# mvenouziou/Boosted_DETR

Measured on AMD Instinct MI355X. Metric: images/sec training step (fwd+matcher+loss+bwd), 640x640 N=100, higher is better.
Workload: dtype f32 (conv/GEMM products as 3 split-f16 [fwd] / split-bf16 [grad] MFMA products, f32 accumulate)

## Files before the change

boosted_detr_amd/_lib.py:

```python
from __future__ import annotations

import ctypes as C
import os
from pathlib import Path

_LIB_PATH = Path(os.environ.get("BDETR_LIB") or Path(__file__).resolve().parent / "csrc" / "libbdetr.so")
_lib = None

c_f32p = C.c_void_p
c_i32p = C.c_void_p
c_i64p = C.c_void_p
c_stream = C.c_void_p


class ConvDesc(C.Structure):
    _fields_ = [(n, C.c_int) for n in ("N", "H", "W", "C", "K", "R", "S", "stride", "pad", "OH", "OW")]


class GemmDesc(C.Structure):
    _fields_ = [
        ("I", C.c_int), ("J", C.c_int), ("R", C.c_int), ("nb0", C.c_int), ("nb1", C.c_int),
        ("a", C.c_void_p), ("lda", C.c_int64), ("sa0", C.c_int64), ("sa1", C.c_int64), ("a_rcontig", C.c_int),
        ("b", C.c_void_p), ("ldb", C.c_int64), ("sb0", C.c_int64), ("sb1", C.c_int64), ("b_rcontig", C.c_int),
        ("c", C.c_void_p), ("ldc", C.c_int64), ("sc0", C.c_int64), ("sc1", C.c_int64),
# ... 101 lines not shown
    "bdetr_debug_checksum": (I, [P, L, P, P, P, I, U64, P]),
    "bdetr_graph_node_census": (I, [P, P, I]),
    "bdetr_bn_stats_fold_rows": (I, []),
    "bdetr_bn_stats_frozen": (I, [P, P, I, F, P, P, P]),
    "bdetr_bn_apply": (I, [P, P, P, P, P, P, I, P, L, I, P]),
    "bdetr_bn_bwd_chunks": (I, [L]),
    "bdetr_bn_bwd": (I, [P, P, P, P, P, P, P, I, I, P, P, P, P, P, L, I, P]),
    "bdetr_bn_rows_stats": (I, [P, I, L, I, F, P, P, P, P, P]),
    "bdetr_bn_rows_apply": (I, [P, P, P, P, P, P, I, L, I, I, P, F, P, P, P, P]),
    "bdetr_bn_rows_bwd": (I, [P, P, P, P, P, I, I, P, P, P, P, I, L, I, P]),
    "bdetr_maxpool3x3s2_fwd": (I, [P, P, I, I, I, I, I, I, P]),
    "bdetr_maxpool3x3s2_bwd": (I, [P, P, P, P, I, I, I, I, I, I, P]),
    "bdetr_stem_pool_bwd_chunks": (I, [L]),
    "bdetr_stem_pool_fwd": (I, [P, P, P, P, P, I, I, I, I, P, P, P, P, P]),
    "bdetr_stem_pool_bwd": (I, [P, P, P, P, P, P, P, I, I, I, I, P, I, P, P, P, P]),
    "bdetr_p16_s2d_pack_bf16": (I, [P, I, I, I, P, P]),
    "bdetr_p16_stem_bwd_weight": (I, [P, P, P, I, I, I, I, P]),
    "bdetr_p16_s2d_unpack_dw": (I, [P, P, I, P]),
    "bdetr_attention_head_dim": (I, []),
    "bdetr_attention_fwd": (I, [P, P, P, P, P, I, I, I, I, F, P]),
    "bdetr_attention_bwd": (I, [P, P, P, P, P, P, P, P, P, P, I, I, I, I, F, P]),
    "bdetr_softmax_rows_fwd": (I, [P, P, L, I, F, P]),
    "bdetr_softmax_rows_bwd": (I, [P, P, P, L, I, F, P]),
    "bdetr_add_dropout_layernorm_fwd": (I, [P, P, P, P, P, P, P, L, I, F, F, U64, P, P]),
    "bdetr_ln_bwd_chunks": (I, [L]),
    "bdetr_add_dropout_layernorm_bwd": (I, [P, P, P, P, P, P, P, P, P, P, P, L, I, F, U64, P, I, P]),
    "bdetr_rowchain_fwd": (I, [C.POINTER(RowchainFwdDesc), P]),
    "bdetr_rowchain_bwd": (I, [C.POINTER(RowchainBwdDesc), P]),
    "bdetr_rowchain_reduce": (I, [P, I, C.POINTER(C.c_void_p * 7), C.POINTER(C.c_int * 7), P]),
    "bdetr_rowchain_width": (I, []),
# ... 88 lines not shown
```

boosted_detr_amd/build.py:

```python
from __future__ import annotations

import hashlib
import os
import subprocess
import sys
from concurrent.futures import ThreadPoolExecutor
from pathlib import Path

CSRC = Path(__file__).resolve().parent / "csrc"
LIB = CSRC / "libbdetr.so"
OBJ_DIR = CSRC / "_obj"
SOURCES = ["common.cpp", "igemm.hip", "sgemm.hip", "hconv.hip", "hwgrad.hip", "p16.hip", "attention.hip", "rowchain.hip", "augment.hip", "norm.hip", "groupnorm_rows.hip", "elementwise.hip", "panoptic.hip", "matcher.hip", "optim.hip", "detmetric.hip", "maskmetric.hip", "maskraster.hip", "maskimage.hip", "panopticmerge.hip"]
ARCH = "gfx950"
COMMON_FLAGS = ["-O3", "-fPIC", f"--offload-arch={ARCH}", "-std=c++20", "-Wall", "-Wno-unused-function"] + os.environ.get("BDETR_CXXFLAGS", "").split()
PER_FILE_FLAGS = {"matcher.hip": ["-ffp-contract=off"], "detmetric.hip": ["-ffp-contract=off"], "maskmetric.hip": ["-ffp-contract=off"],
                  "maskraster.hip": ["-ffp-contract=off"], "maskimage.hip": ["-ffp-contract=off"], "panopticmerge.hip": ["-ffp-contract=off"]}


def _hipcc() -> str:
    for cand in (os.environ.get("HIPCC"), "/opt/rocm/bin/hipcc", "hipcc"):
        if cand and (os.path.isabs(cand) and os.path.exists(cand) or not os.path.isabs(cand)):
            return cand
    raise RuntimeError("hipcc not found")


def _digest(paths) -> str:
    h = hashlib.sha256()
    for p in sorted(paths):
        h.update(p.name.encode())
        h.update(p.read_bytes())
    return h.hexdigest()


def build(force: bool = False, verbose: bool = True) -> Path:
    deps = [CSRC / s for s in SOURCES] + [CSRC / "common.h", CSRC / "gemm_common.h", CSRC / "p16.h", CSRC.parent.parent / "include" / "bdetr.h"]
    stamp = CSRC / "_obj" / "stamp"
    dig = _digest(deps) + "|" + " ".join(COMMON_FLAGS)
    if not force and LIB.exists() and stamp.exists() and stamp.read_text() == dig:
        return LIB
    OBJ_DIR.mkdir(exist_ok=True)
    hipcc = _hipcc()

    headers = [d for d in deps if d.suffix == ".h"]

    def compile_one(src: str) -> Path:
        obj = OBJ_DIR / (src.rsplit(".", 1)[0] + ".o")
        flags = COMMON_FLAGS + PER_FILE_FLAGS.get(src, [])
        ostamp = OBJ_DIR / (src + ".stamp")
        odig = _digest([CSRC / src] + headers) + "|" + " ".join(flags)
        if not force and obj.exists() and ostamp.exists() and ostamp.read_text() == odig:
# ... 22 lines not shown
```

boosted_detr_amd/csrc/norm.hip:

```cpp
#include "common.h"
#include "p16.h"

namespace {

struct ColGeom { int tx, ty, gx; };
inline ColGeom col_geom(int C) {
    int c4 = C / 4;
    int tx = 1; while (tx < c4 && tx < 64) tx <<= 1;
    ColGeom g; g.tx = tx; g.ty = 256 / tx; g.gx = (c4 + tx - 1) / tx; return g;
}

template <class F>
__global__ __launch_bounds__(256) void colreduce2_kernel(F f, int64_t rows, int C, int tx, int64_t rows_per_chunk,
                                                         float* __restrict__ pa, float* __restrict__ pb) {
    __shared__ f32x4 sa[256], sb[256];
    const int tid = threadIdx.x;
    const int cx = tid % tx, ry = tid / tx, ty = 256 / tx;
    const int c = (blockIdx.x * tx + cx) * 4;
    const int64_t r0 = (int64_t)blockIdx.y * rows_per_chunk;
    const int64_t r1 = min(rows, r0 + rows_per_chunk);
    f32x4 a = {0, 0, 0, 0}, b = {0, 0, 0, 0};
    if (c < C) {
        int64_t r = r0 + ry;
        for (; r + ty < r1; r += 2 * ty) {
// ... 176 lines not shown
void sum_partials2(const float* pa, const float* pb, int nparts, int C, float* oa, float* ob, hipStream_t st) {
    if (nparts >= wide_reduce_min() && C % 4 == 0 && (reinterpret_cast<uintptr_t>(pa) | reinterpret_cast<uintptr_t>(pb)) % 16 == 0)
        hipLaunchKernelGGL(reduce_partials2_kernel<false>, dim3(C / 4), dim3(256), 0, st, pa, pb, nparts, C, oa, ob, BnFinalizeArgs{});
    else
        hipLaunchKernelGGL(sum_partials2_kernel, dim3((C + 7) / 8), dim3(256), 0, st, pa, pb, nparts, C, oa, ob);
}

struct StatFn {
    const float* x; int C;
    __device__ __forceinline__ void operator()(int64_t r, int c, f32x4& a, f32x4& b) const {
        f32x4 v = *reinterpret_cast<const f32x4*>(x + r * C + c);
        a = v; b = v * v;
    }
};

__device__ __forceinline__ float bn_affine(float v, float m, float rs, float g, float b) { return __builtin_fmaf(v - m, rs * g, b); }
__device__ __forceinline__ float bn_bwd_dx(float g, float xv, float m, float rs, float gm, float dg, float db, float inv_rows) {
    const float xh = (xv - m) * rs;
    const float t = __builtin_fmaf(-db, inv_rows, g);
    return __builtin_fmaf(-xh, dg * inv_rows, t) * (rs * gm);
}

__device__ __forceinline__ unsigned relu_mask_bits4(const void* mask, int64_t i) {
    const unsigned long long* w = reinterpret_cast<const unsigned long long*>(mask) + (i >> 6) * 4;
    const int b = (int)(i & 63);
    return (unsigned)((w[0] >> b) & 1ull) | ((unsigned)((w[1] >> b) & 1ull) << 1) | ((unsigned)((w[2] >> b) & 1ull) << 2) | ((unsigned)((w[3] >> b) & 1ull) << 3);
}

struct BnBwdFn {
    const float* dout; const float* out; const float* x; const float* mean; const float* rstd; const float* gamma; const float* beta;
    int C; int relu;
    int out_p16 = 0;
    int even_h = 0, even_w = 0;
    int dout_compact = 0;
    __device__ __forceinline__ void operator()(int64_t r, int c, f32x4& a, f32x4& b) const {
        const int64_t rg = r;
// ... 71 lines not shown
            }
        }
        if (dres != nullptr) reinterpret_cast<f32x4*>(dres)[i] = g;
        f32x4 r;
        if (frozen) {
            r = g * (rs * gm);
        } else {
            f32x4 dg = *reinterpret_cast<const f32x4*>(dgamma + c), db = *reinterpret_cast<const f32x4*>(dbeta + c);
#pragma unroll
            for (int e = 0; e < 4; ++e) r[e] = bn_bwd_dx(g[e], xv[e], m[e], rs[e], gm[e], dg[e], db[e], inv_rows);
        }
        reinterpret_cast<f32x4*>(dx)[i] = r;
    }
}

struct StemGeom { int N, H, W, C, PH, PW; };

__global__ __launch_bounds__(256) void stem_pool_fwd_kernel(const float* __restrict__ y, const float* __restrict__ mean, const float* __restrict__ rstd,
                                                            const float* __restrict__ gamma, const float* __restrict__ beta, StemGeom s,
                                                            float* __restrict__ out32, void* __restrict__ out_f16, unsigned* __restrict__ tap,
                                                            int* __restrict__ overflow_flag) {
    const int c4n = s.C / 4;
    const int64_t n4 = (int64_t)s.N * s.PH * s.PW * c4n;
    for (int64_t i = (int64_t)blockIdx.x * blockDim.x + threadIdx.x; i < n4; i += (int64_t)gridDim.x * blockDim.x) {
        const int c4 = (int)(i % c4n); unsigned t = (unsigned)(i / c4n);
        const int pw = (int)(t % (unsigned)s.PW); t /= (unsigned)s.PW; const int ph = (int)(t % (unsigned)s.PH); const int n = (int)(t / (unsigned)s.PH);
        const int c = c4 * 4;
        const f32x4 m = *reinterpret_cast<const f32x4*>(mean + c), rs = *reinterpret_cast<const f32x4*>(rstd + c);
        const f32x4 g = *reinterpret_cast<const f32x4*>(gamma + c), b = *reinterpret_cast<const f32x4*>(beta + c);
        f32x4 v[9];
        bool in[9];
// ... 13 lines not shown
            for (int e = 0; e < 4; ++e) {
                const float a = fmaxf(bn_affine(v[k][e], m[e], rs[e], g[e], b[e]), 0.f);
                if (a > mx[e]) { mx[e] = a; arg = (arg & ~(0xFFu << (8 * e))) | ((unsigned)k << (8 * e)); }
            }
        }
        tap[i] = arg;
        if (out32 != nullptr) reinterpret_cast<f32x4*>(out32)[i] = mx;
        if (out_f16 != nullptr) {
            p16_store4<true>(out_f16, i, mx[0], mx[1], mx[2], mx[3]);
            if (overflow_flag != nullptr) {
                const float top = fmaxf(fmaxf(mx[0], mx[1]), fmaxf(mx[2], mx[3]));
                if (!(top < P16_F16_LIMIT)) *overflow_flag = 1;
            }
        }
    }
}

__device__ __forceinline__ f32x4 stem_pixel_grad(const float* __restrict__ dpool, const unsigned* __restrict__ tap, const StemGeom& s, unsigned px, int c,
                                                 const f32x4 yv, const f32x4 m, const f32x4 rs, const f32x4 gm, const f32x4 bt, f32x4& xhat) {
    const int c4n = s.C / 4, c4 = c / 4;
    const int iw = (int)(px % (unsigned)s.W); const unsigned t = px / (unsigned)s.W;
    const int ih = (int)(t % (unsigned)s.H), n = (int)(t / (unsigned)s.H);
    const int ph0 = ih >> 1, pw0 = iw >> 1;
    const bool two_h = (ih & 1) & (int)(ph0 + 1 < s.PH), two_w = (iw & 1) & (int)(pw0 + 1 < s.PW);
    unsigned word[4];
    f32x4 dv[4];
    unsigned mine[4];
#pragma unroll
    for (int k = 0; k < 4; ++k) {
        const int a = k >> 1, b = k & 1;
        const bool real = (a == 0 || two_h) && (b == 0 || two_w);
        const int ph = ph0 + (a & (int)two_h), pw = pw0 + (b & (int)two_w);
        const int64_t o = (((int64_t)n * s.PH + ph) * s.PW + pw) * c4n + c4;
        mine[k] = real ? (unsigned)((ih - (ph * 2 - 1)) * 3 + (iw - (pw * 2 - 1))) : 0xFFu;
        word[k] = tap[o];
        dv[k] = reinterpret_cast<const f32x4*>(dpool)[o];
    }
    f32x4 g = {0.f, 0.f, 0.f, 0.f};
#pragma unroll
    for (int k = 0; k < 4; ++k)
#pragma unroll
        for (int e = 0; e < 4; ++e) if (((word[k] >> (8 * e)) & 0xFFu) == mine[k]) g[e] += dv[k][e];
    xhat = (yv - m) * rs;
#pragma unroll
    for (int e = 0; e < 4; ++e) if (!(bn_affine(yv[e], m[e], rs[e], gm[e], bt[e]) > 0.f)) g[e] = 0.f;
    return g;
}

struct StemBwdFn {
    const float* dpool; const unsigned* tap; const float* y; const float* mean; const float* rstd; const float* gamma; const float* beta; StemGeom s;
    __device__ __forceinline__ void operator()(int64_t r, int c, f32x4& a, f32x4& b) const {
        const f32x4 yv = *reinterpret_cast<const f32x4*>(y + r * s.C + c);
        const f32x4 m = *reinterpret_cast<const f32x4*>(mean + c), rs = *reinterpret_cast<const f32x4*>(rstd + c);
        const f32x4 gm = *reinterpret_cast<const f32x4*>(gamma + c), bt = *reinterpret_cast<const f32x4*>(beta + c);
        f32x4 xh;
        a = stem_pixel_grad(dpool, tap, s, (unsigned)r, c, yv, m, rs, gm, bt, xh);
        b = a * xh;
    }
};

__global__ __launch_bounds__(256) void stem_bwd_apply_kernel(const float* __restrict__ dpool, const unsigned* __restrict__ tap, const float* __restrict__ y,
// ... 463 lines not shown
    const StemGeom s{N, H, W, C, (H + 2 - 3) / 2 + 1, (W + 2 - 3) / 2 + 1};
    const int64_t rows = (int64_t)N * H * W;
    ColGeom g = col_geom(C);
    int64_t rpc = chunk_rows_for(rows, STEM_BWD_CHUNKS, 64);
    int nch = (int)cdiv64(rows, rpc);
    float* pa = ws; float* pb = ws + (int64_t)nch * C;
    StemBwdFn f{dpool, reinterpret_cast<const unsigned*>(tap), y, mean, rstd, gamma, beta, s};
    hipLaunchKernelGGL((colreduce2_kernel<StemBwdFn>), dim3(g.gx, nch), dim3(256), 0, st, f, rows, C, g.tx, rpc, pa, pb);
    sum_partials2(pa, pb, nch, C, dbeta, dgamma, st);
    const int64_t n4 = rows * C / 4;
    hipLaunchKernelGGL(stem_bwd_apply_kernel, dim3(ew_grid(n4, 256, 2)), dim3(256), 0, st, dpool, reinterpret_cast<const unsigned*>(tap), y, mean, rstd, gamma, beta,
                       dgamma, dbeta, s, dy, dy_p16, n4, 1.0f / (float)rows);
    return bdetr_launch_status("stem_pool_bwd");
}

static int channel_aligned_grid(int64_t n4, int C) {
    int grid = ew_grid(n4, 256, 2);
    int a = C / 4, b = 256;
    while (b) { const int t = a % b; a = b; b = t; }
    const int mult = (C / 4) / a;
    if (mult > 1 && mult <= 8) grid = (grid + mult - 1) / mult * mult;
    return grid;
}

extern "C" int bdetr_bn_apply_p16(const float* x, const float* mean, const float* rstd, const float* gamma,
                                  const float* beta, const void* residual, int residual_p16, const bdetr_bn_affine* residual_bn, int relu,
                                  float* out32, void* out_f16, void* out_bf16,
                                  uint64_t* relu_mask, int* overflow_flag, int64_t rows, int C, void* stream) {
    BDETR_CHECK_ARG(x && mean && rstd && gamma && beta && (out32 || out_f16 || out_bf16) && rows > 0 && C > 0 && C % 8 == 0,
                    "bdetr_bn_apply_p16: bad arguments (C %% 8 == 0 required)");
// ... 142 lines not shown
```

boosted_detr_amd/kernels.py:

```python
from __future__ import annotations

import ctypes as C
from dataclasses import dataclass
from typing import Optional, Tuple

import numpy as np
import torch

from . import _lib
from ._lib import BnAffine, BnBwdFuse, ConvDesc, GemmDesc, LossDesc, RowchainBwdDesc, RowchainFwdDesc, check

ACT_NONE, ACT_RELU, ACT_TANH = 0, 1, 2


_LAUNCH_STREAM = [None]


def set_launch_stream(handle: Optional[int]) -> Optional[int]:
    prev = _LAUNCH_STREAM[0]
    _LAUNCH_STREAM[0] = handle
    return prev


GEMM_FP32, GEMM_BF16X3, GEMM_MIXED, GEMM_SPLIT, GEMM_BF16X6 = 0, 1, 2, 3, 4
# ... 663 lines not shown
                                _p(ws), _stream()), "stem_pool_bwd")
    return dy, dgamma, dbeta


def stem_bwd_weight_s2d(x4, dy_bf16, dw):
    _chk(x4, dy_bf16, dw)
    L = _lib.lib()
    N, H, W, Cc = x4.shape
    Kout = dw.shape[0]
    assert Cc == 4 and H % 2 == 0 and W % 2 == 0 and tuple(dw.shape) == (Kout, 7, 7, 4) and tuple(dy_bf16.shape) == (N, H // 2, W // 2, Kout)
    x2 = empty(N, H // 2, W // 2, 16, like=x4)
    check(L.bdetr_p16_s2d_pack_bf16(_p(x4), N, H, W, _p(x2), _stream()), "p16_s2d_pack_bf16")
    dw2 = empty(Kout, 4, 4, 16, like=x4)
    check(L.bdetr_zero(_p(dw2), dw2.numel(), _stream()), "zero")
    check(L.bdetr_p16_stem_bwd_weight(_p(x2), _p(dy_bf16), _p(dw2), N, H // 2, W // 2, Kout, _stream()), "p16_stem_bwd_weight")
    check(L.bdetr_p16_s2d_unpack_dw(_p(dw2), _p(dw), Kout, _stream()), "p16_s2d_unpack_dw")
    return dw


def attention_fwd(q, k, v, heads, scale):
    _chk(q, k, v)
    B, nq, D = q.shape
    nk = k.shape[1]
    o = empty(B, heads, nq, D // heads, like=q)
    lse = empty(B, heads, nq, like=q)
    check(_lib.lib().bdetr_attention_fwd(_p(q), _p(k), _p(v), _p(o), _p(lse), B, heads, nq, nk, scale, _stream()), "attention_fwd")
    return o, lse


def attention_bwd(q, k, v, o, d_o, lse, heads, scale):
# ... 779 lines not shown
```

boosted_detr_amd/ops.py:

```python
from __future__ import annotations

import math
import os
import weakref
from typing import Optional

import numpy as np
import torch

from . import kernels as K
from . import _lib
from .engine import WEIGHTS_VERSION, Variable, capture, current_tape, dense_contribution, info, materialise, own, side_task, tag

_dropout_site = [0]
_dropout_seed_dev = [None]


def dropout_seed_tensor() -> torch.Tensor:
    if _dropout_seed_dev[0] is None:
        _dropout_seed_dev[0] = torch.full((1,), 0x5EED, dtype=torch.int64, device="cuda")
    return _dropout_seed_dev[0]


def set_dropout_seed(seed: int, write: bool = True) -> None:
# ... 471 lines not shown
        g, mine = g.contiguous(), info(g).owned
        return tuple(own(g[l * B:(l + 1) * B]) if mine else g[l * B:(l + 1) * B] for l in range(L))

    _rec([out], list(xs), backward)
    return out


def maxpool(x: torch.Tensor) -> torch.Tensor:
    y = K.maxpool_fwd(x)
    _rec([y], [x], lambda g: (own(K.maxpool_bwd(x, y, g.contiguous())),))
    return y


STEM_FUSE = os.environ.get("BDETR_STEM_FUSE", "1") != "0"
STEM_S2D = os.environ.get("BDETR_STEM_S2D", "1") != "0"


def conv_bn_relu_maxpool(x: torch.Tensor, w: Variable, b: Variable, bn: BNState, stride: int, pad: int, training: bool,
                         bn_batch_stats: bool) -> torch.Tensor:
    N, H, W, Cin = x.shape
    Kout, R, S, _ = w.value.shape
    if not (STEM_FUSE and training and bn_batch_stats and _p16_active() and Kout % 8 == 0):
        return maxpool(conv_bn(x, w, b, bn, stride, pad, True, training=training, bn_batch_stats=bn_batch_stats, x_needs_grad=False))
    g = K.ConvGeom(N, H, W, Cin, Kout, R, S, stride, pad)
    x32 = as_fp32(x)
    y, parts = K.conv2d_fwd(x32, w.value, b.value, g, K.ACT_NONE, want_stats=True)
    if parts is None or parts[0] is None:
        parts = K.colstats(_2d(y))
    mean, rstd = K.bn_stats(g.M, Kout, parts, bn.eps, bn.momentum, True, bn.moving_mean.value, bn.moving_var.value, like=y)
    _, out, tap = K.stem_pool_fwd(y, mean, rstd, bn.gamma.value, bn.beta.value)
    attach_packed(out, out.detach(), p16_only=True)

    def backward(g_out):
        sg, sb = GradSink(bn.gamma), GradSink(bn.beta)
        s2d = (STEM_S2D and w.needs_grad and (R, S, stride, pad, Cin) == (7, 7, 2, 3, 4) and H % 2 == 0 and W % 2 == 0 and Kout % 64 == 0
               and K.get_gemm_precision() in ("split", "mixed") and not K.deterministic())
        dy, _, _ = K.stem_pool_bwd(materialise(g_out).contiguous(), tap, y, mean, rstd, bn.gamma.value, bn.beta.value, dgamma=sg.buf, dbeta=sb.buf,
                                   dy_p16=s2d)
        sg.commit()
        sb.commit()
        if s2d:
            _param_grads_task(w, b, lambda dw, pz: K.stem_bwd_weight_s2d(x32, dy, dw), None, x32, dy)
        else:
            _param_grads_task(w, b, lambda dw, pz: K.conv2d_bwd_weight(x32, dy, g, dw=dw, prezeroed=pz), None, x32, dy)
        return (None,)

    _rec([out], [x], backward)
    return out


def dense(x: torch.Tensor, w: Variable, b: Variable, act: int = K.ACT_NONE) -> torch.Tensor:
# ... 285 lines not shown
```

include/bdetr.h:

```cpp
#ifndef BDETR_H
#define BDETR_H
#include <stdint.h>
#ifdef __cplusplus
extern "C" {
#endif

#define BDETR_ABI_VERSION 8

int         bdetr_abi_version(void);
const char* bdetr_last_error(void);
int         bdetr_device_cus(void);

int         bdetr_low_priority_stream_create(void** stream_out);
int         bdetr_stream_priority_range(int* least, int* greatest);
int         bdetr_side_stream_candidates(void* main_stream, int ncand, int loads, int ticks, void** streams_out, float* scores_ms, float* unloaded_ms);
int         bdetr_stream_destroy(void* stream);

enum { BDETR_GEMM_FP32 = 0, BDETR_GEMM_BF16X3 = 1, BDETR_GEMM_MIXED = 2, BDETR_GEMM_SPLIT = 3, BDETR_GEMM_BF16X6 = 4 };
int         bdetr_set_gemm_precision(int mode);
int         bdetr_get_gemm_precision(void);

int bdetr_prof_enable(int on);
int bdetr_prof_read(double* total_ms, int64_t* launches, double* flops);
int bdetr_prof_read_arith(int arith, double* total_ms, int64_t* launches, double* flops);
// ... 128 lines not shown
                      int grouped_stats, int frozen, float* dx, float* dgamma, float* dbeta, float* ws, int G, int64_t R, int C,
                      void* stream);

int bdetr_maxpool3x3s2_fwd(const float* x, float* y, int N, int H, int W, int C, int OH, int OW, void* stream);
int bdetr_maxpool3x3s2_bwd(const float* x, const float* y, const float* dy, float* dx,
                           int N, int H, int W, int C, int OH, int OW, void* stream);

int bdetr_stem_pool_bwd_chunks(int64_t rows);
int bdetr_stem_pool_fwd(const float* y, const float* mean, const float* rstd, const float* gamma, const float* beta,
                        int N, int H, int W, int C, float* out32, void* out_f16, uint8_t* tap, int* overflow_flag, void* stream);
int bdetr_stem_pool_bwd(const float* dpool, const uint8_t* tap, const float* y, const float* mean, const float* rstd, const float* gamma,
                        const float* beta, int N, int H, int W, int C, float* dy, int dy_p16 , float* dgamma, float* dbeta, float* ws, void* stream);
int bdetr_p16_s2d_pack_bf16(const float* x, int N, int H, int W, void* out_bf16, void* stream);
int bdetr_p16_stem_bwd_weight(const void* x2_bf16, const void* dy_bf16, float* dw2, int N, int H2, int W2, int K, void* stream);
int bdetr_p16_s2d_unpack_dw(const float* dw2, float* dw, int K, void* stream);

int bdetr_softmax_rows_fwd(const float* s, float* p, int64_t rows, int cols, float scale, void* stream);
int bdetr_softmax_rows_bwd(const float* p, const float* dp, float* ds, int64_t rows, int cols, float scale, void* stream);

int bdetr_attention_head_dim(void);
int bdetr_attention_fwd(const float* q, const float* k, const float* v, float* o, float* lse,
                        int B, int h, int nq, int nk, float scale, void* stream);
int bdetr_attention_bwd(const float* q, const float* k, const float* v, const float* o, const float* d_o,
                        const float* lse, float* dq, float* dk, float* dv, float* dvec_ws,
                        int B, int h, int nq, int nk, float scale, void* stream);

int bdetr_add_dropout_layernorm_fwd(const float* x, const float* y, const float* gamma, const float* beta,
                                    float* out, float* mean, float* rstd, int64_t rows, int D,
                                    float eps, float rate, uint64_t seed, const uint64_t* seed_base, void* stream);
int bdetr_ln_bwd_chunks(int64_t rows);
// ... 162 lines not shown
```

Before: 649.2.

## Fuse stem maxpool/BN/ReLU backward into stem weight-gradient GEMM

Adds a fused kernel for the stem conv weight gradient. It recomputes the maxpool/ReLU/BN backward dy on the fly from dpool, the tap indices and y, splits it into bf16 hi/lo, and feeds it straight into MFMA with the space-to-depth input. A separate column-reduction kernel now computes only dgamma/dbeta. This removes writing and re-reading the full stem dy tensor, at the cost of reading dpool/tap/y twice (once for the sums, once in the GEMM) and atomic accumulation of the output.

Measured after the change: 652.6, median of 6. No clear change (+0.5%).

```diff
diff --git a/boosted_detr_amd/_lib.py b/boosted_detr_amd/_lib.py
--- a/boosted_detr_amd/_lib.py
+++ b/boosted_detr_amd/_lib.py
@@ -139,6 +139,8 @@
     "bdetr_stem_pool_bwd_chunks": (I, [L]),
     "bdetr_stem_pool_fwd": (I, [P, P, P, P, P, I, I, I, I, P, P, P, P, P]),
     "bdetr_stem_pool_bwd": (I, [P, P, P, P, P, P, P, I, I, I, I, P, I, P, P, P, P]),
+    "bdetr_stem_pool_bwd_sums": (I, [P, P, P, P, P, P, P, I, I, I, I, P, P, P, P]),
+    "bdetr_stem_bwd_weight_fused": (I, [P, P, P, P, P, P, P, P, P, P, P, I, I, I, I, P]),
     "bdetr_p16_s2d_pack_bf16": (I, [P, I, I, I, P, P]),
     "bdetr_p16_stem_bwd_weight": (I, [P, P, P, I, I, I, I, P]),
     "bdetr_p16_s2d_unpack_dw": (I, [P, P, I, P]),
diff --git a/boosted_detr_amd/build.py b/boosted_detr_amd/build.py
--- a/boosted_detr_amd/build.py
+++ b/boosted_detr_amd/build.py
@@ -10,7 +10,7 @@
 CSRC = Path(__file__).resolve().parent / "csrc"
 LIB = CSRC / "libbdetr.so"
 OBJ_DIR = CSRC / "_obj"
-SOURCES = ["common.cpp", "igemm.hip", "sgemm.hip", "hconv.hip", "hwgrad.hip", "p16.hip", "attention.hip", "rowchain.hip", "augment.hip", "norm.hip", "groupnorm_rows.hip", "elementwise.hip", "panoptic.hip", "matcher.hip", "optim.hip", "detmetric.hip", "maskmetric.hip", "maskraster.hip", "maskimage.hip", "panopticmerge.hip"]
+SOURCES = ["common.cpp", "igemm.hip", "sgemm.hip", "hconv.hip", "hwgrad.hip", "p16.hip", "attention.hip", "rowchain.hip", "augment.hip", "norm.hip", "stemwgrad.hip", "groupnorm_rows.hip", "elementwise.hip", "panoptic.hip", "matcher.hip", "optim.hip", "detmetric.hip", "maskmetric.hip", "maskraster.hip", "maskimage.hip", "panopticmerge.hip"]
 ARCH = "gfx950"
 COMMON_FLAGS = ["-O3", "-fPIC", f"--offload-arch={ARCH}", "-std=c++20", "-Wall", "-Wno-unused-function"] + os.environ.get("BDETR_CXXFLAGS", "").split()
 PER_FILE_FLAGS = {"matcher.hip": ["-ffp-contract=off"], "detmetric.hip": ["-ffp-contract=off"], "maskmetric.hip": ["-ffp-contract=off"],
@@ -33,7 +33,7 @@
 
 
 def build(force: bool = False, verbose: bool = True) -> Path:
-    deps = [CSRC / s for s in SOURCES] + [CSRC / "common.h", CSRC / "gemm_common.h", CSRC / "p16.h", CSRC.parent.parent / "include" / "bdetr.h"]
+    deps = [CSRC / s for s in SOURCES] + [CSRC / "common.h", CSRC / "gemm_common.h", CSRC / "p16.h", CSRC / "stem_bn.h", CSRC.parent.parent / "include" / "bdetr.h"]
     stamp = CSRC / "_obj" / "stamp"
     dig = _digest(deps) + "|" + " ".join(COMMON_FLAGS)
     if not force and LIB.exists() and stamp.exists() and stamp.read_text() == dig:
diff --git a/boosted_detr_amd/csrc/norm.hip b/boosted_detr_amd/csrc/norm.hip
--- a/boosted_detr_amd/csrc/norm.hip
+++ b/boosted_detr_amd/csrc/norm.hip
@@ -1,5 +1,6 @@
 #include "common.h"
 #include "p16.h"
+#include "stem_bn.h"
 
 namespace {
 
@@ -214,12 +215,6 @@
     }
 };
 
-__device__ __forceinline__ float bn_affine(float v, float m, float rs, float g, float b) { return __builtin_fmaf(v - m, rs * g, b); }
-__device__ __forceinline__ float bn_bwd_dx(float g, float xv, float m, float rs, float gm, float dg, float db, float inv_rows) {
-    const float xh = (xv - m) * rs;
-    const float t = __builtin_fmaf(-db, inv_rows, g);
-    return __builtin_fmaf(-xh, dg * inv_rows, t) * (rs * gm);
-}
 
 __device__ __forceinline__ unsigned relu_mask_bits4(const void* mask, int64_t i) {
     const unsigned long long* w = reinterpret_cast<const unsigned long long*>(mask) + (i >> 6) * 4;
@@ -321,7 +316,6 @@
     }
 }
 
-struct StemGeom { int N, H, W, C, PH, PW; };
 
 __global__ __launch_bounds__(256) void stem_pool_fwd_kernel(const float* __restrict__ y, const float* __restrict__ mean, const float* __restrict__ rstd,
                                                             const float* __restrict__ gamma, const float* __restrict__ beta, StemGeom s,
@@ -365,37 +359,6 @@
             }
         }
     }
-}
-
-__device__ __forceinline__ f32x4 stem_pixel_grad(const float* __restrict__ dpool, const unsigned* __restrict__ tap, const StemGeom& s, unsigned px, int c,
-                                                 const f32x4 yv, const f32x4 m, const f32x4 rs, const f32x4 gm, const f32x4 bt, f32x4& xhat) {
-    const int c4n = s.C / 4, c4 = c / 4;
-    const int iw = (int)(px % (unsigned)s.W); const unsigned t = px / (unsigned)s.W;
-    const int ih = (int)(t % (unsigned)s.H), n = (int)(t / (unsigned)s.H);
-    const int ph0 = ih >> 1, pw0 = iw >> 1;
-    const bool two_h = (ih & 1) & (int)(ph0 + 1 < s.PH), two_w = (iw & 1) & (int)(pw0 + 1 < s.PW);
-    unsigned word[4];
-    f32x4 dv[4];
-    unsigned mine[4];
-#pragma unroll
-    for (int k = 0; k < 4; ++k) {
-        const int a = k >> 1, b = k & 1;
-        const bool real = (a == 0 || two_h) && (b == 0 || two_w);
-        const int ph = ph0 + (a & (int)two_h), pw = pw0 + (b & (int)two_w);
-        const int64_t o = (((int64_t)n * s.PH + ph) * s.PW + pw) * c4n + c4;
-        mine[k] = real ? (unsigned)((ih - (ph * 2 - 1)) * 3 + (iw - (pw * 2 - 1))) : 0xFFu;
-        word[k] = tap[o];
-        dv[k] = reinterpret_cast<const f32x4*>(dpool)[o];
-    }
-    f32x4 g = {0.f, 0.f, 0.f, 0.f};
-#pragma unroll
-    for (int k = 0; k < 4; ++k)
-#pragma unroll
-        for (int e = 0; e < 4; ++e) if (((word[k] >> (8 * e)) & 0xFFu) == mine[k]) g[e] += dv[k][e];
-    xhat = (yv - m) * rs;
-#pragma unroll
-    for (int e = 0; e < 4; ++e) if (!(bn_affine(yv[e], m[e], rs[e], gm[e], bt[e]) > 0.f)) g[e] = 0.f;
-    return g;
 }
 
 struct StemBwdFn {
@@ -889,6 +852,24 @@
     return bdetr_launch_status("stem_pool_bwd");
 }
 
+extern "C" int bdetr_stem_pool_bwd_sums(const float* dpool, const uint8_t* tap, const float* y, const float* mean, const float* rstd, const float* gamma,
+                                        const float* beta, int N, int H, int W, int C, float* dgamma, float* dbeta, float* ws, void* stream) {
+    BDETR_CHECK_ARG(dpool && tap && y && mean && rstd && gamma && beta && dgamma && dbeta && ws && N > 0 && H > 0 && W > 0 && C > 0 && C % 8 == 0,
+                    "bdetr_stem_pool_bwd_sums: bad arguments (C %% 8 == 0 required)");
+    BDETR_CHECK_ARG((int64_t)N * H * W < (int64_t)1 << 31, "bdetr_stem_pool_bwd_sums: more than 2^31 pixels");
+    hipStream_t st = (hipStream_t)stream;
+    const StemGeom s{N, H, W, C, (H + 2 - 3) / 2 + 1, (W + 2 - 3) / 2 + 1};
+    const int64_t rows = (int64_t)N * H * W;
+    ColGeom g = col_geom(C);
+    int64_t rpc = chunk_rows_for(rows, STEM_BWD_CHUNKS, 64);
+    int nch = (int)cdiv64(rows, rpc);
+    float* pa = ws; float* pb = ws + (int64_t)nch * C;
+    StemBwdFn f{dpool, reinterpret_cast<const unsigned*>(tap), y, mean, rstd, gamma, beta, s};
+    hipLaunchKernelGGL((colreduce2_kernel<StemBwdFn>), dim3(g.gx, nch), dim3(256), 0, st, f, rows, C, g.tx, rpc, pa, pb);
+    sum_partials2(pa, pb, nch, C, dbeta, dgamma, st);
+    return bdetr_launch_status("stem_pool_bwd_sums");
+}
+
 static int channel_aligned_grid(int64_t n4, int C) {
     int grid = ew_grid(n4, 256, 2);
     int a = C / 4, b = 256;
diff --git a/boosted_detr_amd/csrc/stem_bn.h b/boosted_detr_amd/csrc/stem_bn.h
--- /dev/null
+++ b/boosted_detr_amd/csrc/stem_bn.h
@@ -0,0 +1,76 @@
+#pragma once
+#include "common.h"
+
+__device__ __forceinline__ float bn_affine(float v, float m, float rs, float g, float b) { return __builtin_fmaf(v - m, rs * g, b); }
+__device__ __forceinline__ float bn_bwd_dx(float g, float xv, float m, float rs, float gm, float dg, float db, float inv_rows) {
+    const float xh = (xv - m) * rs;
+    const float t = __builtin_fmaf(-db, inv_rows, g);
+    return __builtin_fmaf(-xh, dg * inv_rows, t) * (rs * gm);
+}
+
+struct StemGeom { int N, H, W, C, PH, PW; };
+
+__device__ __forceinline__ f32x4 stem_pixel_grad(const float* __restrict__ dpool, const unsigned* __restrict__ tap, const StemGeom& s, unsigned px, int c,
+                                                 const f32x4 yv, const f32x4 m, const f32x4 rs, const f32x4 gm, const f32x4 bt, f32x4& xhat) {
+    const int c4n = s.C / 4, c4 = c / 4;
+    const int iw = (int)(px % (unsigned)s.W); const unsigned t = px / (unsigned)s.W;
+    const int ih = (int)(t % (unsigned)s.H), n = (int)(t / (unsigned)s.H);
+    const int ph0 = ih >> 1, pw0 = iw >> 1;
+    const bool two_h = (ih & 1) & (int)(ph0 + 1 < s.PH), two_w = (iw & 1) & (int)(pw0 + 1 < s.PW);
+    unsigned word[4];
+    f32x4 dv[4];
+    unsigned mine[4];
+#pragma unroll
+    for (int k = 0; k < 4; ++k) {
+        const int a = k >> 1, b = k & 1;
+        const bool real = (a == 0 || two_h) && (b == 0 || two_w);
+        const int ph = ph0 + (a & (int)two_h), pw = pw0 + (b & (int)two_w);
+        const int64_t o = (((int64_t)n * s.PH + ph) * s.PW + pw) * c4n + c4;
+        mine[k] = real ? (unsigned)((ih - (ph * 2 - 1)) * 3 + (iw - (pw * 2 - 1))) : 0xFFu;
+        word[k] = tap[o];
+        dv[k] = reinterpret_cast<const f32x4*>(dpool)[o];
+    }
+    f32x4 g = {0.f, 0.f, 0.f, 0.f};
+#pragma unroll
+    for (int k = 0; k < 4; ++k)
+#pragma unroll
+        for (int e = 0; e < 4; ++e) if (((word[k] >> (8 * e)) & 0xFFu) == mine[k]) g[e] += dv[k][e];
+    xhat = (yv - m) * rs;
+#pragma unroll
+    for (int e = 0; e < 4; ++e) if (!(bn_affine(yv[e], m[e], rs[e], gm[e], bt[e]) > 0.f)) g[e] = 0.f;
+    return g;
+}
+
+struct StemTaps { unsigned word[4]; f32x4 dv[4]; };
+__device__ __forceinline__ void stem_pixel_taps(const float* __restrict__ dpool, const unsigned* __restrict__ tap, const StemGeom& s, int n, int ih, int iw,
+                                                int c, StemTaps& t) {
+    const int c4n = s.C / 4, c4 = c / 4;
+    const int ph0 = ih >> 1, pw0 = iw >> 1;
+    const bool two_h = (ih & 1) & (int)(ph0 + 1 < s.PH), two_w = (iw & 1) & (int)(pw0 + 1 < s.PW);
+#pragma unroll
+    for (int k = 0; k < 4; ++k) {
+        const int a = k >> 1, b = k & 1;
+        const int ph = ph0 + (a & (int)two_h), pw = pw0 + (b & (int)two_w);
+        const int64_t o = (((int64_t)n * s.PH + ph) * s.PW + pw) * c4n + c4;
+        t.word[k] = tap[o];
+        t.dv[k] = reinterpret_cast<const f32x4*>(dpool)[o];
+    }
+}
+__device__ __forceinline__ f32x4 stem_pixel_grad_taps(const StemTaps& t, const StemGeom& s, int ih, int iw, const f32x4 yv, const f32x4 m, const f32x4 rs,
+                                                      const f32x4 gm, const f32x4 bt) {
+    const int ph0 = ih >> 1, pw0 = iw >> 1;
+    const bool two_h = (ih & 1) & (int)(ph0 + 1 < s.PH), two_w = (iw & 1) & (int)(pw0 + 1 < s.PW);
+    f32x4 g = {0.f, 0.f, 0.f, 0.f};
+#pragma unroll
+    for (int k = 0; k < 4; ++k) {
+        const int a = k >> 1, b = k & 1;
+        const bool real = (a == 0 || two_h) && (b == 0 || two_w);
+        const int ph = ph0 + (a & (int)two_h), pw = pw0 + (b & (int)two_w);
+        const unsigned mine = real ? (unsigned)((ih - (ph * 2 - 1)) * 3 + (iw - (pw * 2 - 1))) : 0xFFu;
+#pragma unroll
+        for (int e = 0; e < 4; ++e) if (((t.word[k] >> (8 * e)) & 0xFFu) == mine) g[e] += t.dv[k][e];
+    }
+#pragma unroll
+    for (int e = 0; e < 4; ++e) if (!(bn_affine(yv[e], m[e], rs[e], gm[e], bt[e]) > 0.f)) g[e] = 0.f;
+    return g;
+}
diff --git a/boosted_detr_amd/csrc/stemwgrad.hip b/boosted_detr_amd/csrc/stemwgrad.hip
--- /dev/null
+++ b/boosted_detr_amd/csrc/stemwgrad.hip
@@ -0,0 +1,235 @@
+#include "gemm_common.h"
+#include "p16.h"
+#include "stem_bn.h"
+
+namespace {
+
+constexpr int BK = 32;
+constexpr int BM = 64, BN = 256;
+constexpr int NW = 4, NT = NW * 64;
+constexpr int A_BYTES = BM * 128, B_BYTES = BN * 128, STAGE_BYTES = A_BYTES + B_BYTES;
+constexpr int A_ROW = BM * 4, B_ROW = BN * 4;
+constexpr unsigned OOB = 0xFFFFFFF0u;
+constexpr unsigned NUM_RECORDS = 0xFFFFFF00u;
+
+typedef __bf16 bf16x8 __attribute__((ext_vector_type(8)));
+typedef unsigned int u32x4 __attribute__((ext_vector_type(4)));
+typedef unsigned int u32x2 __attribute__((ext_vector_type(2)));
+typedef __attribute__((address_space(3))) void lds_void;
+
+__device__ __forceinline__ int xx_swz(int r) { return ((r & 1) << 3) | ((r >> 1) & 1); }
+
+struct StemWgradArgs {
+    const float* dpool; const unsigned* tap; const float* y;
+    const float* mean; const float* rstd; const float* gamma; const float* beta; const float* dgamma; const float* dbeta;
+    const void* x2; float* dw2;
+    StemGeom s;
+    int M, r_chunk;
+    float inv_rows;
+};
+
+__global__ __launch_bounds__(NT, 2) void stem_wgrad_fused_kernel(StemWgradArgs p) {
+    __shared__ __attribute__((aligned(16))) unsigned char lds[2 * STAGE_BYTES];
+    const int tid = threadIdx.x, lane = tid & 63;
+    const int wave = __builtin_amdgcn_readfirstlane(tid >> 6);
+    const int H = p.s.H, W = p.s.W;
+    const int r_begin = (int)blockIdx.x * p.r_chunk, r_end = min(p.M, r_begin + p.r_chunk);
+    const int nk = (r_end - r_begin + BK - 1) / BK;
+
+    const int c4 = tid & 15, c = c4 * 4;
+    const f32x4 m = *reinterpret_cast<const f32x4*>(p.mean + c), rs = *reinterpret_cast<const f32x4*>(p.rstd + c);
+    const f32x4 gm = *reinterpret_cast<const f32x4*>(p.gamma + c), bt = *reinterpret_cast<const f32x4*>(p.beta + c);
+    const f32x4 dg = *reinterpret_cast<const f32x4*>(p.dgamma + c), db = *reinterpret_cast<const f32x4*>(p.dbeta + c);
+    int an[2], aih[2], aiw[2];
+    unsigned a_lds[2];
+#pragma unroll
+    for (int j = 0; j < 2; ++j) {
+        const int r = (tid >> 4) + 16 * j;
+        const unsigned px = (unsigned)(r_begin + r);
+        aiw[j] = (int)(px % (unsigned)W); const unsigned t = px / (unsigned)W;
+        aih[j] = (int)(t % (unsigned)H); an[j] = (int)(t / (unsigned)H);
+        a_lds[j] = (unsigned)(r * A_ROW + (((2 * (c4 >> 1)) ^ xx_swz(r)) * 16) + 8 * (c4 & 1));
+    }
+    const int d_ow = BK % W, d_oh = BK / W;
+    StemTaps taps[2]; f32x4 yv[2];
+    auto a_load = [&](int kt) {
+#pragma unroll
+        for (int j = 0; j < 2; ++j) {
+            const int r = r_begin + kt * BK + (tid >> 4) + 16 * j;
+            const bool in = r < r_end;
+            int n = an[j], ih = aih[j], iw = aiw[j];
+            if (!in) {
+                const unsigned px = (unsigned)(r_end - 1);
+                iw = (int)(px % (unsigned)W); const unsigned t = px / (unsigned)W;
+                ih = (int)(t % (unsigned)H); n = (int)(t / (unsigned)H);
+                an[j] = n; aih[j] = ih; aiw[j] = iw;
+            }
+            const int64_t px = ((int64_t)n * H + ih) * W + iw;
+            yv[j] = reinterpret_cast<const f32x4*>(p.y)[px * 16 + c4];
+            stem_pixel_taps(p.dpool, p.tap, p.s, n, ih, iw, c, taps[j]);
+        }
+    };
+    auto a_store = [&](int kt, int buf) {
+#pragma unroll
+        for (int j = 0; j < 2; ++j) {
+            const bool in = r_begin + kt * BK + (tid >> 4) + 16 * j < r_end;
+            const f32x4 g = stem_pixel_grad_taps(taps[j], p.s, aih[j], aiw[j], yv[j], m, rs, gm, bt);
+            float v[4];
+#pragma unroll
+            for (int e = 0; e < 4; ++e) v[e] = in ? bn_bwd_dx(g[e], yv[j][e], m[e], rs[e], gm[e], dg[e], db[e], p.inv_rows) : 0.f;
+            unsigned h01, l01, h23, l23;
+            p16_split2_bf16(v[0], v[1], h01, l01);
+            p16_split2_bf16(v[2], v[3], h23, l23);
+            unsigned char* q = lds + buf * STAGE_BYTES;
+            *reinterpret_cast<u32x2*>(q + a_lds[j]) = u32x2{h01, h23};
+            *reinterpret_cast<u32x2*>(q + (a_lds[j] ^ 16u)) = u32x2{l01, l23};
+            if (in) {
+                aiw[j] += d_ow; aih[j] += d_oh;
+                if (aiw[j] >= W) { aiw[j] -= W; ++aih[j]; }
+                while (aih[j] >= H) { aih[j] -= H; ++an[j]; }
+            }
+        }
+    };
+
+    const unsigned long long xa = reinterpret_cast<unsigned long long>(p.x2);
+    const unsigned xlo = __builtin_amdgcn_readfirstlane((unsigned)xa), xhi = __builtin_amdgcn_readfirstlane((unsigned)(xa >> 32));
+    const __amdgpu_buffer_rsrc_t rsB = __builtin_amdgcn_make_buffer_rsrc(reinterpret_cast<void*>(((unsigned long long)xhi << 32) | xlo), 0, (int)NUM_RECORDS, 0x00020000);
+    const int chunk = lane ^ xx_swz(wave);
+    const int x8 = chunk >> 1, btap = x8 >> 1, btr = btap >> 2, bts = btap & 3;
+    const unsigned b_lane = (unsigned)(((btr - 2) * W + (bts - 2)) * 64 + (x8 & 1) * 32 + (chunk & 1) * 16);
+    int boh[8], bow[8];
+#pragma unroll
+    for (int t = 0; t < 8; ++t) {
+        const unsigned px = (unsigned)(r_begin + 4 * t + wave);
+        bow[t] = (int)(px % (unsigned)W); boh[t] = (int)((px / (unsigned)W) % (unsigned)H);
+    }
+    auto b_issue = [&](int kt, int buf) {
+#pragma unroll
+        for (int t = 0; t < 8; ++t) {
+            const int r = r_begin + kt * BK + 4 * t + wave;
+            const bool ok = r < r_end && (unsigned)(boh[t] + btr - 2) < (unsigned)H && (unsigned)(bow[t] + bts - 2) < (unsigned)W;
+            const unsigned vo = ok ? (unsigned)r * 64u + b_lane : OOB;
+            __builtin_amdgcn_raw_ptr_buffer_load_lds(rsB, (lds_void*)(lds + buf * STAGE_BYTES + A_BYTES + (4 * t + wave) * B_ROW), 16, (int)vo, 0, 0, 0);
+            bow[t] += d_ow; boh[t] += d_oh;
+            if (bow[t] >= W) { bow[t] -= W; ++boh[t]; }
+            while (boh[t] >= H) boh[t] -= H;
+        }
+    };
+
+    f32x16 acc[2][2];
+    {
+        float z = 0.f;
+        asm volatile("" : "+v"(z));
+#pragma unroll
+        for (int a = 0; a < 2; ++a)
+#pragma unroll
+            for (int b = 0; b < 2; ++b)
+#pragma unroll
+                for (int e = 0; e < 16; ++e) acc[a][b][e] = z;
+    }
+    const int lh = lane >> 5, li = lane & 31;
+    unsigned fa_h[2], fa_l[2], fb_h[2], fb_l[2];
+    {
+        const int g16 = (lane >> 4) & 1, q = (lane >> 2) & 3, pp = lane & 3;
+        const int r0 = 8 * lh + q;
+        const unsigned lds0 = (unsigned)(size_t)(__attribute__((address_space(3))) const unsigned char*)lds;
+#pragma unroll
+        for (int i = 0; i < 2; ++i) {
+            const int ua = (i * 32 + 16 * g16 + 4 * pp) >> 3, ub = (wave * 64 + i * 32 + 16 * g16 + 4 * pp) >> 3;
+            const int sa = (2 * ua) ^ xx_swz(r0), sb = (2 * ub) ^ xx_swz(r0);
+            const unsigned basea = lds0 + (unsigned)(r0 * A_ROW + 8 * (pp & 1)), baseb = lds0 + (unsigned)(A_BYTES + r0 * B_ROW + 8 * (pp & 1));
+            fa_h[i] = basea + (unsigned)(sa * 16); fa_l[i] = basea + (unsigned)((sa ^ 1) * 16);
+            fb_h[i] = baseb + (unsigned)(sb * 16); fb_l[i] = baseb + (unsigned)((sb ^ 1) * 16);
+        }
+    }
+    auto half = [&](int buf, auto ks_c) {
+        constexpr int ks = decltype(ks_c)::value;
+        constexpr int a0 = ks * 16 * A_ROW, a1 = a0 + 4 * A_ROW, b0 = ks * 16 * B_ROW, b1 = b0 + 4 * B_ROW;
+        static_assert(b1 < 65536, "ds offset field");
+        const unsigned so = (unsigned)(buf * STAGE_BYTES);
+        const unsigned pah0 = fa_h[0] + so, pal0 = fa_l[0] + so, pah1 = fa_h[1] + so, pal1 = fa_l[1] + so;
+        const unsigned pbh0 = fb_h[0] + so, pbl0 = fb_l[0] + so, pbh1 = fb_h[1] + so, pbl1 = fb_l[1] + so;
+        u32x2 ah0x, ah0y, al0x, al0y, ah1x, ah1y, al1x, al1y, bh0x, bh0y, bl0x, bl0y, bh1x, bh1y, bl1x, bl1y;
+        asm volatile(
+            "ds_read_b64_tr_b16 %0, %16 offset:%24\n\t"
+            "ds_read_b64_tr_b16 %1, %16 offset:%25\n\t"
+            "ds_read_b64_tr_b16 %2, %17 offset:%24\n\t"
+            "ds_read_b64_tr_b16 %3, %17 offset:%25\n\t"
+            "ds_read_b64_tr_b16 %4, %18 offset:%24\n\t"
+            "ds_read_b64_tr_b16 %5, %18 offset:%25\n\t"
+            "ds_read_b64_tr_b16 %6, %19 offset:%24\n\t"
+            "ds_read_b64_tr_b16 %7, %19 offset:%25\n\t"
+            "ds_read_b64_tr_b16 %8, %20 offset:%26\n\t"
+            "ds_read_b64_tr_b16 %9, %20 offset:%27\n\t"
+            "ds_read_b64_tr_b16 %10, %21 offset:%26\n\t"
+            "ds_read_b64_tr_b16 %11, %21 offset:%27\n\t"
+            "ds_read_b64_tr_b16 %12, %22 offset:%26\n\t"
+            "ds_read_b64_tr_b16 %13, %22 offset:%27\n\t"
+            "ds_read_b64_tr_b16 %14, %23 offset:%26\n\t"
+            "ds_read_b64_tr_b16 %15, %23 offset:%27\n\t"
+            "s_waitcnt lgkmcnt(0)"
+            : "=&v"(ah0x), "=&v"(ah0y), "=&v"(al0x), "=&v"(al0y), "=&v"(ah1x), "=&v"(ah1y), "=&v"(al1x), "=&v"(al1y),
+              "=&v"(bh0x), "=&v"(bh0y), "=&v"(bl0x), "=&v"(bl0y), "=&v"(bh1x), "=&v"(bh1y), "=&v"(bl1x), "=&v"(bl1y)
+            : "v"(pah0), "v"(pal0), "v"(pah1), "v"(pal1), "v"(pbh0), "v"(pbl0), "v"(pbh1), "v"(pbl1), "n"(a0), "n"(a1), "n"(b0), "n"(b1)
+            : "memory");
+        const u32x4 ah[2] = {u32x4{ah0x[0], ah0x[1], ah0y[0], ah0y[1]}, u32x4{ah1x[0], ah1x[1], ah1y[0], ah1y[1]}};
+        const u32x4 al[2] = {u32x4{al0x[0], al0x[1], al0y[0], al0y[1]}, u32x4{al1x[0], al1x[1], al1y[0], al1y[1]}};
+        const u32x4 bh[2] = {u32x4{bh0x[0], bh0x[1], bh0y[0], bh0y[1]}, u32x4{bh1x[0], bh1x[1], bh1y[0], bh1y[1]}};
+        const u32x4 bl[2] = {u32x4{bl0x[0], bl0x[1], bl0y[0], bl0y[1]}, u32x4{bl1x[0], bl1x[1], bl1y[0], bl1y[1]}};
+#define BF8(v) __builtin_bit_cast(bf16x8, v)
+#pragma unroll
+        for (int a = 0; a < 2; ++a)
+#pragma unroll
+            for (int b = 0; b < 2; ++b) {
+                acc[a][b] = __builtin_amdgcn_mfma_f32_32x32x16_bf16(BF8(al[a]), BF8(bh[b]), acc[a][b], 0, 0, 0);
+                acc[a][b] = __builtin_amdgcn_mfma_f32_32x32x16_bf16(BF8(ah[a]), BF8(bl[b]), acc[a][b], 0, 0, 0);
+                acc[a][b] = __builtin_amdgcn_mfma_f32_32x32x16_bf16(BF8(ah[a]), BF8(bh[b]), acc[a][b], 0, 0, 0);
+            }
+#undef BF8
+    };
+
+    if (nk > 0) { b_issue(0, 0); a_load(0); a_store(0, 0); }
+    for (int kt = 0; kt < nk; ++kt) {
+        const int buf = kt & 1;
+        asm volatile("s_waitcnt vmcnt(0) lgkmcnt(0)\n\ts_barrier" ::: "memory");
+        const bool more = kt + 1 < nk;
+        if (more) { b_issue(kt + 1, buf ^ 1); a_load(kt + 1); }
+        half(buf, std::integral_constant<int, 0>{});
+        half(buf, std::integral_constant<int, 1>{});
+        if (more) a_store(kt + 1, buf ^ 1);
+    }
+
+#pragma unroll
+    for (int a = 0; a < 2; ++a)
+#pragma unroll
+        for (int b = 0; b < 2; ++b)
+#pragma unroll
+            for (int e = 0; e < 16; ++e) {
+                const int row = a * 32 + (e & 3) + 8 * (e >> 2) + 4 * lh, col = wave * 64 + b * 32 + li;
+                const float v = acc[a][b][e];
+                unsafeAtomicAdd(p.dw2 + row * BN + col, v);
+            }
+}
+
+}
+
+extern "C" int bdetr_stem_bwd_weight_fused(const float* dpool, const uint8_t* tap, const float* y, const float* mean, const float* rstd, const float* gamma,
+                                           const float* beta, const float* dgamma, const float* dbeta, const void* x2_bf16, float* dw2,
+                                           int N, int H, int W, int K, void* stream) {
+    BDETR_CHECK_ARG(dpool && tap && y && mean && rstd && gamma && beta && dgamma && dbeta && x2_bf16 && dw2 && N > 0 && H > 0 && W > 0 && K == 64,
+                    "bdetr_stem_bwd_weight_fused: bad arguments (K == 64)");
+    BDETR_CHECK_ARG(reinterpret_cast<uintptr_t>(x2_bf16) % 16 == 0 && reinterpret_cast<uintptr_t>(y) % 16 == 0 && reinterpret_cast<uintptr_t>(dpool) % 16 == 0,
+                    "bdetr_stem_bwd_weight_fused: unaligned tensor");
+    const int64_t M64 = (int64_t)N * H * W;
+    BDETR_CHECK_ARG(M64 * 64 < (int64_t)NUM_RECORDS && M64 < (1LL << 31) - 2 * BK, "bdetr_stem_bwd_weight_fused: x2 of 4 GB or more");
+    StemWgradArgs a{dpool, reinterpret_cast<const unsigned*>(tap), y, mean, rstd, gamma, beta, dgamma, dbeta, x2_bf16, dw2,
+                    StemGeom{N, H, W, K, (H + 2 - 3) / 2 + 1, (W + 2 - 3) / 2 + 1}, (int)M64, 0, 1.0f / (float)M64};
+    int64_t sk = 2LL * bdgemm::num_cus();
+    const int64_t maxsk = cdiv64(M64, 8LL * BK);
+    if (sk > maxsk) sk = maxsk;
+    if (sk < 1) sk = 1;
+    a.r_chunk = (int)(cdiv64(cdiv64(M64, sk), BK) * BK);
+    const int grid = (int)cdiv64(M64, a.r_chunk);
+    hipLaunchKernelGGL(stem_wgrad_fused_kernel, dim3(grid), dim3(NT), 0, (hipStream_t)stream, a);
+    return bdetr_launch_status("stem_bwd_weight_fused");
+}
diff --git a/boosted_detr_amd/kernels.py b/boosted_detr_amd/kernels.py
--- a/boosted_detr_amd/kernels.py
+++ b/boosted_detr_amd/kernels.py
@@ -701,6 +701,36 @@
     dw2 = empty(Kout, 4, 4, 16, like=x4)
     check(L.bdetr_zero(_p(dw2), dw2.numel(), _stream()), "zero")
     check(L.bdetr_p16_stem_bwd_weight(_p(x2), _p(dy_bf16), _p(dw2), N, H // 2, W // 2, Kout, _stream()), "p16_stem_bwd_weight")
+    check(L.bdetr_p16_s2d_unpack_dw(_p(dw2), _p(dw), Kout, _stream()), "p16_s2d_unpack_dw")
+    return dw
+
+
+def stem_pool_bwd_sums(dpool, tap, y, mean, rstd, gamma, beta, dgamma=None, dbeta=None):
+    _chk(dpool, y, mean, rstd, gamma, beta, dgamma, dbeta)
+    assert tap.is_cuda and tap.is_contiguous() and tap.dtype == torch.uint8 and tuple(tap.shape) == tuple(dpool.shape)
+    L = _lib.lib()
+    N, H, W, Cc = y.shape
+    dgamma = empty(Cc, like=y) if dgamma is None else dgamma
+    dbeta = empty(Cc, like=y) if dbeta is None else dbeta
+    ws = empty(2 * Cc * L.bdetr_stem_pool_bwd_chunks(N * H * W), like=y)
+    check(L.bdetr_stem_pool_bwd_sums(_p(dpool), _p(tap), _p(y), _p(mean), _p(rstd), _p(gamma), _p(beta), N, H, W, Cc, _p(dgamma), _p(dbeta), _p(ws),
+                                     _stream()), "stem_pool_bwd_sums")
+    return dgamma, dbeta
+
+
+def stem_bwd_weight_fused(dpool, tap, y, mean, rstd, gamma, beta, dgamma, dbeta, x4, dw):
+    _chk(dpool, y, mean, rstd, gamma, beta, dgamma, dbeta, x4, dw)
+    assert tap.is_cuda and tap.is_contiguous() and tap.dtype == torch.uint8 and tuple(tap.shape) == tuple(dpool.shape)
+    L = _lib.lib()
+    N, H, W, Cc = x4.shape
+    Kout = dw.shape[0]
+    assert Cc == 4 and H % 2 == 0 and W % 2 == 0 and Kout == 64 and tuple(dw.shape) == (Kout, 7, 7, 4) and tuple(y.shape) == (N, H // 2, W // 2, Kout)
+    x2 = empty(N, H // 2, W // 2, 16, like=x4)
+    check(L.bdetr_p16_s2d_pack_bf16(_p(x4), N, H, W, _p(x2), _stream()), "p16_s2d_pack_bf16")
+    dw2 = empty(Kout, 4, 4, 16, like=x4)
+    check(L.bdetr_zero(_p(dw2), dw2.numel(), _stream()), "zero")
+    check(L.bdetr_stem_bwd_weight_fused(_p(dpool), _p(tap), _p(y), _p(mean), _p(rstd), _p(gamma), _p(beta), _p(dgamma), _p(dbeta), _p(x2), _p(dw2),
+                                        N, H // 2, W // 2, Kout, _stream()), "stem_bwd_weight_fused")
     check(L.bdetr_p16_s2d_unpack_dw(_p(dw2), _p(dw), Kout, _stream()), "p16_s2d_unpack_dw")
     return dw
 
diff --git a/boosted_detr_amd/ops.py b/boosted_detr_amd/ops.py
--- a/boosted_detr_amd/ops.py
+++ b/boosted_detr_amd/ops.py
@@ -509,6 +509,7 @@
 
 STEM_FUSE = os.environ.get("BDETR_STEM_FUSE", "1") != "0"
 STEM_S2D = os.environ.get("BDETR_STEM_S2D", "1") != "0"
+STEM_WGRAD_FUSE = os.environ.get("BDETR_STEM_WGRAD_FUSE", "1") != "0"
 
 
 def conv_bn_relu_maxpool(x: torch.Tensor, w: Variable, b: Variable, bn: BNState, stride: int, pad: int, training: bool,
@@ -530,6 +531,14 @@
         sg, sb = GradSink(bn.gamma), GradSink(bn.beta)
         s2d = (STEM_S2D and w.needs_grad and (R, S, stride, pad, Cin) == (7, 7, 2, 3, 4) and H % 2 == 0 and W % 2 == 0 and Kout % 64 == 0
                and K.get_gemm_precision() in ("split", "mixed") and not K.deterministic())
+        if s2d and STEM_WGRAD_FUSE and Kout == 64:
+            dpool = materialise(g_out).contiguous()
+            K.stem_pool_bwd_sums(dpool, tap, y, mean, rstd, bn.gamma.value, bn.beta.value, dgamma=sg.buf, dbeta=sb.buf)
+            sg.commit()
+            sb.commit()
+            _write_param_grads(w, b, lambda dw, pz: K.stem_bwd_weight_fused(dpool, tap, y, mean, rstd, bn.gamma.value, bn.beta.value, sg.buf, sb.buf,
+                                                                            x32, dw), None)
+            return (None,)
         dy, _, _ = K.stem_pool_bwd(materialise(g_out).contiguous(), tap, y, mean, rstd, bn.gamma.value, bn.beta.value, dgamma=sg.buf, dbeta=sb.buf,
                                    dy_p16=s2d)
         sg.commit()
diff --git a/include/bdetr.h b/include/bdetr.h
--- a/include/bdetr.h
+++ b/include/bdetr.h
@@ -166,6 +166,11 @@
 int bdetr_p16_s2d_pack_bf16(const float* x, int N, int H, int W, void* out_bf16, void* stream);
 int bdetr_p16_stem_bwd_weight(const void* x2_bf16, const void* dy_bf16, float* dw2, int N, int H2, int W2, int K, void* stream);
 int bdetr_p16_s2d_unpack_dw(const float* dw2, float* dw, int K, void* stream);
+int bdetr_stem_pool_bwd_sums(const float* dpool, const uint8_t* tap, const float* y, const float* mean, const float* rstd, const float* gamma,
+                             const float* beta, int N, int H, int W, int C, float* dgamma, float* dbeta, float* ws, void* stream);
+int bdetr_stem_bwd_weight_fused(const float* dpool, const uint8_t* tap, const float* y, const float* mean, const float* rstd, const float* gamma,
+                                const float* beta, const float* dgamma, const float* dbeta, const void* x2_bf16, float* dw2,
+                                int N, int H, int W , int K , void* stream);
 
 int bdetr_softmax_rows_fwd(const float* s, float* p, int64_t rows, int cols, float scale, void* stream);
 int bdetr_softmax_rows_bwd(const float* p, const float* dp, float* ds, int64_t rows, int cols, float scale, void* stream);
```
